# jinggqu/NextGen-UIA

Hardware: AMD Instinct MI355X
Metric: images/sec fwd+bwd BiomedCLIP+Mona bs=256 (higher is better)
Workload: dtype bf16

## Files before the change

### nextgen-uia_amd/csrc/gemm.hip

```cpp
#include "gemm_epilogue.h"

int uia_gemm_quad_launch(hipStream_t stream, const UiaGemmParams& p, bool specialise, int xflags);
int uia_gemm_quadv_launch(hipStream_t stream, const UiaGemmParams& p, bool specialise, int xflags, int depth);

namespace {

template <typename T, int BM, int BN, int WAVES_M, int WAVES_N>
__global__ __launch_bounds__(64 * WAVES_M * WAVES_N) void gemm_tn_kernel(const UiaGemmParams p) {
    extern __shared__ __attribute__((aligned(16))) char smem[];
    constexpr int NW = WAVES_M * WAVES_N;
    constexpr int WTM = BM / WAVES_M, WTN = BN / WAVES_N;
    constexpr int MT = WTM / 16, NT = WTN / 16;
    constexpr int A_BYTES = BM * 128, W_BYTES = BN * 128, BUF_BYTES = A_BYTES + W_BYTES;
    constexpr int A_PER_WAVE = (BM / 8) / NW, W_PER_WAVE = (BN / 8) / NW;
    static_assert((BM / 8) % NW == 0 && (BN / 8) % NW == 0, "staging must divide over the waves");
    static_assert(WTM % 16 == 0 && WTN % 16 == 0 && (NT % 2) == 0, "wave tile shape");
    constexpr int ESZ = (int)sizeof(T);

    const int tid = threadIdx.x, lane = tid & 63;
    const int wave = __builtin_amdgcn_readfirstlane(tid >> 6);
    const int wm = wave / WAVES_N, wn = wave % WAVES_N;

    const int tiles_n = (p.N + BN - 1) / BN;
    const int nwg = gridDim.x;
    int bid = blockIdx.x;
    {
// ... 1201 lines not shown
                  "uia_gemm: outT_kb_rows needs outT, at least M rows, N*sizeof(T) a multiple of 64 and no row remapping");
    UIA_CHECK_ARG(!p.resid_ln_stats || p.resid_ln_dim >= 0, "uia_gemm: resid_ln_dim=%d", p.resid_ln_dim);
    UIA_CHECK_ARG(!p.rowsum_out || ((uintptr_t)p.rowsum_out % 16 == 0 && p.out_group == 0), "uia_gemm: rowsum_out must be 16-byte aligned and takes no row remapping");
    UIA_CHECK_ARG(!(p.resid_ln_stats && p.resid_ln_dim > 0) || (uintptr_t)p.resid_ln_stats % 16 == 0, "uia_gemm: row sums behind resid_ln_stats must be 16-byte aligned");
    UIA_CHECK_ARG(!p.ln_flag || (uintptr_t)p.ln_flag % 4 == 0, "uia_gemm: ln_flag must be a 4-byte aligned device word");
    UIA_CHECK_ARG(p.drop_where >= 0 && p.drop_where <= 2, "uia_gemm: drop_where=%d (0 none, 1 A operand, 2 accumulator)", p.drop_where);
    UIA_CHECK_ARG(p.drop_where == 0 || (p.drop_p >= 0.f && p.drop_p < 1.f), "uia_gemm: drop_p=%f outside [0, 1)", (double)p.drop_p);
    UIA_CHECK_ARG(p.drop_where != 1 || (dtype == UIA_BF16 && (size_t)p.M * (size_t)p.K / 8 <= 0xFFFFFFFFull && (uintptr_t)p.a_drop_out % 16 == 0 && !p.a_kb_rows),
                  "uia_gemm: dropout on the A operand needs bf16, row-major A, M*K <= 2^35 and a 16-byte aligned a_drop_out");
    UIA_CHECK_ARG(p.drop_where != 2 || (size_t)p.M * (size_t)p.N / 8 <= 0xFFFFFFFFull, "uia_gemm: dropout on the accumulator needs M*N <= 2^35");
    UIA_CHECK_ARG(p.drop_where == 1 || !p.a_drop_out, "uia_gemm: a_drop_out without drop_where = 1");
    UIA_CHECK_ARG(p.K2 >= 0 && (p.K2 == 0 || (dtype == UIA_BF16 && p.A2 && p.K2 % 32 == 0 && p.K2 < p.K && p.lda2 >= p.K2 && (p.lda2 * 2) % 16 == 0 && (uintptr_t)p.A2 % 16 == 0 &&
                                             p.a2_group_cols >= 0 && p.a2_group_cols % 256 == 0 && !p.a_kb_rows && p.lda >= p.K - p.K2)),
                  "uia_gemm: the K extension needs bf16, a row-major A of K - K2 columns, a 16-byte aligned row-major A2 with K2 (a multiple of 32, < K) columns and "
                  "column groups that are multiples of 256; got K=%d K2=%d lda2=%lld group=%d", p.K, p.K2, (long long)p.lda2, p.a2_group_cols);
    UIA_CHECK_ARG(!p.lnfold_sums || (p.lnfold_colsum && p.lnfold_dim > 0 && p.alpha == 1.0f && (uintptr_t)p.lnfold_sums % 16 == 0 && (uintptr_t)p.lnfold_colsum % 16 == 0),
                  "uia_gemm: lnfold_sums needs lnfold_colsum (16-byte aligned), lnfold_dim > 0 and alpha == 1");
    UIA_CHECK_ARG(!p.outT || p.outT_kb_rows || p.ldo >= p.N, "uia_gemm: ldo=%lld < N=%d", (long long)p.ldo, p.N);
    UIA_CHECK_ARG(!p.out32 || p.ldo32 >= p.N, "uia_gemm: ldo32=%lld < N=%d", (long long)p.ldo32, p.N);
    UIA_CHECK_ARG(!p.aux_out || p.ldaux_out >= p.N, "uia_gemm: ldaux_out=%lld < N=%d", (long long)p.ldaux_out, p.N);
    UIA_CHECK_ARG(!p.aux_in || p.ldaux_in >= p.N, "uia_gemm: ldaux_in=%lld < N=%d", (long long)p.ldaux_in, p.N);
    UIA_CHECK_ARG(!p.resid || p.ldr >= p.N, "uia_gemm: ldr=%lld < N=%d", (long long)p.ldr, p.N);
    UIA_CHECK_ARG(!p.residT || p.residT_kb_rows || p.ldrT >= p.N, "uia_gemm: ldrT=%lld < N=%d", (long long)p.ldrT, p.N);
    if (dtype == UIA_BF16) return launch_typed<bf16_t>(stream, p, cfg);
    return launch_typed<float>(stream, p, cfg);
}
```

### nextgen-uia_amd/uia_hip/functional.py

```python
import math
import os
import weakref

import time

import torch

from . import handoff, ops
from ._lib import UiaError
from .handoff import (ClsGrad, Resid3, _g3_partner_feeds, cls_grad_of, fwd3_of, grad3_decode, grad3_of, grad_resid3_enabled, hook_free, linear_chain,
                      publish_cls_grad, publish_fwd3, publish_grad3, publish_rows, publish_t_copy, set_cls_grad, set_grad_resid3, t_copy_of, take_rows, zero_sums,
                      cls_only, set_cls_forward, take_cls_forward)
from .handoff import clear as clear_t_copies

_STATE = {"dtype": torch.bfloat16, "seed": 0x5EED, "calls": 0, "fwd_resid3": os.environ.get("UIA_FWD_RESID3", "1") != "0"}


def set_compute_dtype(dt):
    assert dt in (torch.bfloat16, torch.float32)
    _STATE["dtype"] = dt


def compute_dtype():
    return _STATE["dtype"]
# ... 300 lines not shown
WEIGHTS = WeightCache()


def _empty(shape, dt, like):
    return torch.empty(shape, device=like.device, dtype=dt)


def _act(M, K, dt, like, n_consumer):
    if ops.kb_ok(M, n_consumer, K, dt):
        return ops.kb_empty(M, K, dt, like.device)
    return torch.empty((M, K), device=like.device, dtype=dt)


def _attn_act(M, K, dt, like, n_consumer):
    return _act(M, K, dt, like, n_consumer) if dt == torch.bfloat16 else torch.empty((M, K), device=like.device, dtype=dt)


def _as_act(buf, M, K, dt, n_consumer):
    if ops.kb_ok(M, n_consumer, K, dt):
        return buf if ops.is_kb(buf) else ops.KBlocked.over(buf.view(M, K))
    return buf.as_rows() if ops.is_kb(buf) else buf


def _rows_tile_cfg(m_dense, w, like, dt, **facts):
    if dt != torch.float32 or not like.is_cuda:
        return 0
    N, K = (w.row if isinstance(w, ops.PackedW) else w).shape
    plan = ops.plan_gemm(m_dense, N, K, 4, ops.num_cus(like.device.index), 0, packed=isinstance(w, ops.PackedW), **facts)
    return next(L.base for L in plan if L.lo == 0)


MONA_PARAM_ORDER = ("gamma", "gammax", "project1.weight", "project1.bias", "project2.weight", "project2.bias", "norm.weight", "norm.bias",
                    "adapter_conv.conv1.weight", "adapter_conv.conv1.bias", "adapter_conv.conv2.weight", "adapter_conv.conv2.bias",
                    "adapter_conv.conv3.weight", "adapter_conv.conv3.bias", "adapter_conv.projector.weight", "adapter_conv.projector.bias",
                    "adapter_conv.freq_filter", "adapter_conv.noise_estimator.1.weight", "adapter_conv.noise_estimator.1.bias",
                    "adapter_conv.noise_estimator.3.weight", "adapter_conv.noise_estimator.3.bias")
_SPATIAL_MAP = {"adapter_conv.conv1.weight": "conv1_w", "adapter_conv.conv1.bias": "conv1_b", "adapter_conv.conv2.weight": "conv2_w",
                "adapter_conv.conv2.bias": "conv2_b", "adapter_conv.conv3.weight": "conv3_w", "adapter_conv.conv3.bias": "conv3_b",
                "adapter_conv.projector.weight": "proj_w", "adapter_conv.projector.bias": "proj_b", "adapter_conv.freq_filter": "freq",
                "adapter_conv.noise_estimator.1.weight": "ne1_w", "adapter_conv.noise_estimator.1.bias": "ne1_b",
                "adapter_conv.noise_estimator.3.weight": "ne3_w", "adapter_conv.noise_estimator.3.bias": "ne3_b"}


class MonaFn(torch.autograd.Function):

    @staticmethod
    def forward(ctx, x, variant, hw, p_drop, keep_mask, names, direct, *params):
        P = dict(zip(names, params))
        B, N, D = x.shape
# ... 8 lines not shown
        sp = {_SPATIAL_MAP[k]: v.detach().contiguous() for k, v in P.items() if k in _SPATIAL_MAP}
        seed = _next_seed() if (p_drop > 0 and keep_mask is None) else 0
        fold = not rows and ln_fold_enabled(dt, M)
        if not rows and ops.mona_fused_ok(dt, D, h, w, bott):
            train = any(ctx.needs_input_grad)
            u = _empty((M, D), dt, x) if train else None
            t = _empty((M, bott), dt, x) if train else None
            d = _empty((M, bott), dt, x) if train else None
            w1, w2 = WEIGHTS.get(P["project1.weight"], dt), WEIGHTS.get(P["project2.weight"], dt)
            y = torch.empty_like(x)
            y_t, sums = (_act(M, D, dt, x, 3 * D), zero_sums(M, x.device)) if fold else (None, None)
            ops.mona_fused_fwd(variant, B, h, w, x, P["norm.weight"], P["norm.bias"], P["gamma"], P["gammax"], w1.row, P["project1.bias"], w2.row,
                               P["project2.bias"], sp, y, y_t=y_t, rowsum=sums, u_out=u, t_out=t, d_out=d, p_drop=p_drop, seed=seed, keep_mask=keep_mask)
            if fold:
                publish_rows(y, y_t, sums)
        else:
            u = _empty((M, D), dt, x)
            w1 = WEIGHTS.get(P["project1.weight"], dt)
            t = _empty((M, bott), dt, x)
            if ops.MONA_PRE_FWD_T and x.is_cuda and dt == torch.bfloat16 and D == 768 and bott == 64:
                ops.mona_pre_fwd(x, P["norm.weight"], P["norm.bias"], P["gamma"], P["gammax"], u, proj1=(w1.row if isinstance(w1, ops.PackedW) else w1, P["project1.bias"], t))
            else:
                ops.mona_pre_fwd(x, P["norm.weight"], P["norm.bias"], P["gamma"], P["gammax"], u)
                ops.gemm(u, w1, bias=P["project1.bias"], out_t=t, tile_cfg=_rows_tile_cfg(B * ntok, w1, x, dt, out_t=True) if rows else 0)
            d = _empty((M, bott), dt, x)
            if rows:
                ops.mona_cls_fwd(B, ntok, t, d, p_drop=p_drop, seed=seed, keep_mask=keep_mask)
            else:
                ops.mona_spatial_fwd(variant, B, h, w, t, sp, d, p_drop=p_drop, seed=seed, keep_mask=keep_mask)
            w2 = WEIGHTS.get(P["project2.weight"], dt)
            y = torch.empty_like(x)
            y_t, sums = (_act(M, D, dt, x, 3 * D), zero_sums(M, x.device)) if fold else (None, None)
            three = fold and dt == torch.bfloat16 and _STATE.get("fwd_resid3", True) and handoff.fwd3_consumer_ahead() and M > 2048 and x.is_cuda
            y_lo = torch.empty(M, D, device=x.device, dtype=torch.int8) if three else None
            ops.gemm(d, w2, bias=P["project2.bias"], resid=x.view(M, D), out32=None if three else y.view(M, D), out_t=y_t, out_lo=y_lo, rowsum=sums,
                     tile_cfg=_rows_tile_cfg(B * ntok, w2, x, dt, out32=True, resid=True) if rows else 0)
            if three:
                y = publish_fwd3(x.shape, x.device, y_t, y_lo, sums)
            elif fold:
                publish_rows(y, y_t, sums)
        if u is not None:
            ctx.save_for_backward(x, u, t, d, keep_mask if keep_mask is not None else x.new_empty(0), *params)
        ctx.meta = (variant, hw, p_drop, seed, names, keep_mask is not None)
        ctx.direct_params = tuple(params) if direct else None
        ctx.g3_out = dt == torch.bfloat16 and _g3_partner_feeds(x)
        front = handoff.partner_node(x)
        ctx.cls_ok = not rows and u is not None and type(front).__name__ == "VitBlockFnBackward" and handoff.takes_cls_grad(x)
        ctx.rows_ntok = ntok if rows else 0
        return y

    @staticmethod
    def backward_cls(ctx, cg):
        ntok = getattr(ctx, "rows_ntok", 0)
        variant, hw, p_drop, seed, names, has_mask = ctx.meta
        x, u, t, d, keep_mask, *params = ctx.saved_tensors
        keep_mask = keep_mask if has_mask else None
        P = dict(zip(names, params))
        B, N, D = x.shape
        dt, bott = u.dtype, t.shape[1]
        dy = cg.rows32
        dy_t = dy if dt == torch.float32 else (cg.rows_t if cg.rows_t is not None else t_copy_of(dy, dt))
        direct = ctx.direct_params is not None and all(_is_flat_grad(p) for p in ctx.direct_params)
        G = ({k: p.grad for k, p in zip(names, ctx.direct_params)} if direct
             else {k: torch.zeros_like(v, dtype=torch.float32) for k, v in P.items()})
        cls_rows = lambda a: a.view(B, N * a.shape[1])[:, :a.shape[1]]
        side = _wgrad_side_stream(x.device) if _STATE.get("wgrad_side_stream", False) else None
        w2t = WEIGHTS.get(P["project2.weight"], dt, transpose=True)
        dd = _empty((B, bott), dt, x)
        _wgrad_beside(side, lambda: ops.gemm(dy_t, w2t, out_t=dd), dy_t, cls_rows(d), G["project2.weight"], G["project2.bias"])
        dtt = _empty((B, bott), dt, x)
        ops.mona_cls_bwd(B, ntok or N, dd, t, dtt, p_drop=p_drop, seed=seed, keep_mask=keep_mask, t_rows=bool(ntok))
        w1t = WEIGHTS.get(P["project1.weight"], dt, transpose=True)
        fuse_du = x.is_cuda and ops.mona_pre_bwd_du_ok(B, D, bott, dt)
        du = None if fuse_du else _empty((B, D), dt, x)
        _wgrad_beside(side, None if fuse_du else (lambda: ops.gemm(dtt, w1t, out_t=du)), dtt, cls_rows(u), G["project1.weight"], G["project1.bias"])
        need_dx = ctx.needs_input_grad[0]
        x_cls = x.view(B, D) if ntok else ops.copy_rows(x.view(B * N, D), N, _empty((B, D), torch.float32, x))
        dx = _empty((B, D), torch.float32, x) if need_dx else None
        dx_t = _empty((B, D), dt, x) if (need_dx and dt != torch.float32) else None
        w1t_rows = (dtt, w1t.row if isinstance(w1t, ops.PackedW) else w1t) if fuse_du else None
        ops.mona_pre_bwd(du, x_cls, dy if need_dx else None, P["norm.weight"], P["norm.bias"], P["gamma"], P["gammax"], dx, dx_t,
                         G["gamma"], G["gammax"], G["norm.weight"], G["norm.bias"], dt_w1t=w1t_rows)
        if need_dx and ntok:
            dx = dx.view(B, 1, D)
            publish_t_copy(dx, dx_t.view(B, 1, D) if dx_t is not None else None)
        elif need_dx:
            dx = publish_cls_grad(x.shape, x.device, dx, dx_t) if ctx.cls_ok else ClsGrad(dx, dx_t, N).decode()
        grads = tuple(None if direct else (G[k] if ctx.needs_input_grad[7 + i] else None) for i, k in enumerate(names))
        return (dx, None, None, None, None, None, None) + grads

    @staticmethod
    def backward(ctx, dy):
        if getattr(ctx, "rows_ntok", 0):
            dy = dy.contiguous()
            B, _, D = dy.shape
            dt = ctx.saved_tensors[1].dtype
            return MonaFn.backward_cls(ctx, ClsGrad(dy.view(B, D), t_copy_of(dy, dt).view(B, D) if dt != torch.float32 else None, ctx.rows_ntok))
        cg = cls_grad_of(dy)
# ... 186 lines not shown
            saved, ctx.layout = handoff.save_layout(x3.resid3 if x3 is not None else x, qkv, a, lse, Resid3(h1, lo1) if r3 else x1, pre)
            ctx.save_for_backward(*saved)
            ctx.xshape = (B, N, D)
            ctx.spec = spec
            ctx.g3_out = dt == torch.bfloat16 and _g3_partner_feeds(x)
            ctx.cls_ok = spec.mask is None and N <= ATTN_SINGLE_PASS_MAX and D == 64 * spec.heads and not r3 and handoff.cls_grad_enabled()
        return x2

    @staticmethod
    def _forward_cls(ctx, x, x3, qkv, spec, shape, dt, train):
        B, N, D = shape
        like = qkv
        a = _empty((B, D), dt, like)
        lse = torch.empty(B, spec.heads, device=like.device, dtype=torch.float32) if train else None
        ops.attn_fwd_cls(qkv[:, :D], qkv[:, D:2 * D], qkv[:, 2 * D:], a, B, spec.heads, N, lse=lse)
        x_cls = torch.empty(B, D, device=like.device, dtype=torch.float32)
        if x3 is not None:
            ops.rows3_to_f32(x3.hi, x3.lo, N, x_cls)
        else:
            ops.copy_rows(x.view(B * N, D), N, x_cls)
        x1 = torch.empty(B, D, device=like.device, dtype=torch.float32)
        M = B * N
        wp = WEIGHTS.get(spec.proj[0], dt)
        ops.gemm(a, wp, bias=spec.proj[1], resid=x_cls, out32=x1, tile_cfg=_rows_tile_cfg(M, wp, like, dt, out32=True, resid=True))
        h2 = _empty((B, D), dt, like)
        ops.layernorm_fwd(x1, spec.ln2[0], spec.ln2[1], spec.eps, y_t=h2)
        F = spec.fc1[0].shape[0]
        f = _empty((B, F), dt, like)
        pre = _empty((B, F), dt, like) if train else None
        w1, w2 = WEIGHTS.get(spec.fc1[0], dt), WEIGHTS.get(spec.fc2[0], dt)
        ops.gemm(h2, w1, bias=spec.fc1[1], act=spec.act, aux_out=pre, out_t=f, tile_cfg=_rows_tile_cfg(M, w1, like, dt, act=True, aux_out=train, out_t=True))
        x2 = torch.empty(B, 1, D, device=like.device, dtype=torch.float32)
        ops.gemm(f, w2, bias=spec.fc2[1], resid=x1, out32=x2.view(B, D), tile_cfg=_rows_tile_cfg(M, w2, like, dt, out32=True, resid=True))
        if train:
            saved, ctx.layout = handoff.save_layout(x3.resid3 if x3 is not None else x, qkv, a, lse, x1, pre)
            ctx.save_for_backward(*saved)
            ctx.xshape = (B, N, D)
            ctx.spec = spec
            ctx.g3_out = dt == torch.bfloat16 and _g3_partner_feeds(x)
            ctx.cls_ok = False
            ctx.cls_fwd = True
        handoff.cls_rows_out(True)
        return x2

    @staticmethod
    def backward_cls(ctx, cg):
        compact = getattr(ctx, "cls_fwd", False)
        xin, qkv, a, lse, x1, pre = handoff.restore_layout(ctx.saved_tensors, ctx.layout)
        x3_in = isinstance(xin, Resid3)
        x = xin.lo if x3_in else xin
        spec = ctx.spec
        B, N, D = ctx.xshape
        M, dt = B * N, qkv.dtype
        F = pre.shape[1]
        dy = cg.rows32
        dy_t = dy if dt == torch.float32 else (cg.rows_t if cg.rows_t is not None else t_copy_of(dy, dt))
        pre_cls = pre if compact else ops.copy_rows(pre, N, _empty((B, F), dt, x))
        dpre = _empty((B, F), dt, x)
        ops.gemm(dy_t, WEIGHTS.get(spec.fc2[0], dt, transpose=True), dact=spec.act, aux_in=pre_cls, out_t=dpre)
        dh = _empty((B, D), dt, x)
        ops.gemm(dpre, WEIGHTS.get(spec.fc1[0], dt, transpose=True), out_t=dh)
        x1_cls = x1 if compact else ops.copy_rows(x1, N, _empty((B, D), torch.float32, x))
        dx1 = _empty((B, D), torch.float32, x)
        dx1_t = _empty((B, D), dt, x) if dt != torch.float32 else dx1
        ops.layernorm_bwd(dh, x1_cls, spec.ln2[0], spec.eps, dres=dy, dx32=dx1, dx_t=dx1_t if dt != torch.float32 else None)
        da = dh
        ops.gemm(dx1_t, WEIGHTS.get(spec.proj[0], dt, transpose=True), out_t=da)
        dqkv = _attn_act(M, 3 * D, dt, x, D)
        if ops.is_kb(dqkv):
            ops.attn_bwd_cls(qkv[:, :D], qkv[:, D:2 * D], qkv[:, 2 * D:], a, da, lse, dqkv, None, None, B, spec.heads, N, rows=compact)
        else:
            ops.attn_bwd_cls(qkv[:, :D], qkv[:, D:2 * D], qkv[:, 2 * D:], a, da, lse, dqkv[:, :D], dqkv[:, D:2 * D], dqkv[:, 2 * D:], B, spec.heads, N, rows=compact)
        dh1 = _empty((M, D), dt, x)
        ops.gemm(dqkv, WEIGHTS.get(spec.qkv[0], dt, transpose=True), out_t=dh1)
        xrows = xin if x3_in else x.view(M, D)
        if getattr(ctx, "g3_out", False):
            dx_t = _empty((M, D), dt, x)
            dlo = torch.empty(M, D, device=x.device, dtype=torch.int8)
            ops.layernorm_bwd_periodic(dh1, xrows, spec.ln1[0], spec.eps, dx1, N, dx_t=dx_t, dx_lo=dlo)
            return publish_grad3((B, N, D), x.device, dx_t, dlo), None
        dx = torch.empty(B, N, D, device=x.device, dtype=torch.float32)
        if dt == torch.float32:
            ops.layernorm_bwd_periodic(dh1, xrows, spec.ln1[0], spec.eps, dx1, N, dx32=dx.view(M, D))
            return dx, None
        dx_t = _empty((M, D), dt, x)
        ops.layernorm_bwd(dh1, xrows, spec.ln1[0], spec.eps, dres=ClsGrad(dx1, None, N).decode().view(M, D), dx32=dx.view(M, D), dx_t=dx_t)
        publish_t_copy(dx, dx_t)
        return dx, None

    @staticmethod
# ... 99 lines not shown
    rows = torch.empty(B, D, device=res.w.device, dtype=torch.float32)
    if res.lo is not None:
        ops.rows3_to_f32(res.hi, res.lo, L, rows)
    else:
        ops.copy_rows(res.raw.view(-1, D), L, rows)
        if res.stats is None:
            return rows
    ops.layernorm_fwd(rows, res.w, res.b, res.eps if res.eps is not None else eps, y32=rows)
    return rows


def post_ln_layer_cls_ok(x_t, heads, L, cu_seqlens=None):
    D = x_t.cols if ops.is_kb(x_t) else x_t.shape[1]
    return cu_seqlens is None and D == 64 * heads and 1 < L <= 288 and x_t.is_cuda and not (x_t.dtype != torch.float32 and _STATE.get("text_resid_t", False))


def _post_ln_layer_cls(res, qkv, L, B, heads, P, keylen, eps, D, dt):
    a = _empty((B, D), dt, qkv)
    ops.attn_fwd_cls(qkv[:, :D], qkv[:, D:2 * D], qkv[:, 2 * D:], a, B, heads, L, mask="keypad", keylen=keylen)
    r = _res_cls_rows(res, L, B, D, eps)
    s_a = torch.empty(B, D, device=qkv.device, dtype=torch.float32)
    M = B * L
    wo = WEIGHTS.get(P["attention.output.dense.weight"], dt)
    ops.gemm(a, wo, bias=P["attention.output.dense.bias"], resid=r, out32=s_a, tile_cfg=_rows_tile_cfg(M, wo, qkv, dt, out32=True, resid=True))
    h = _empty((B, D), dt, qkv)
    ops.layernorm_fwd(s_a, P["attention.output.LayerNorm.weight"], P["attention.output.LayerNorm.bias"], eps, y_t=h, y32=s_a)
    F = P["intermediate.dense.weight"].shape[0]
    f = _empty((B, F), dt, qkv)
    w1, w2 = WEIGHTS.get(P["intermediate.dense.weight"], dt), WEIGHTS.get(P["output.dense.weight"], dt)
    ops.gemm(h, w1, bias=P["intermediate.dense.bias"], act="gelu", out_t=f, tile_cfg=_rows_tile_cfg(M, w1, qkv, dt, act=True, out_t=True))
    ops.gemm(f, w2, bias=P["output.dense.bias"], resid=s_a, out32=r, tile_cfg=_rows_tile_cfg(M, w2, qkv, dt, out32=True, resid=True))
    ops.layernorm_fwd(r, P["output.LayerNorm.weight"], P["output.LayerNorm.bias"], eps, y_t=h, y32=r)
    return LnResidual(r, None, P["output.LayerNorm.weight"], P["output.LayerNorm.bias"]), h


def post_ln_layer(res, x_t, L, B, heads, P, keylen, eps=1e-12, cu_seqlens=None, fold_sums=None, fold_out=False, cls_only=False):
    kb_in = ops.is_kb(x_t)
    M, D = (x_t.rows, x_t.cols) if kb_in else x_t.shape
    dt = x_t.dtype
    t_resid = dt != torch.float32 and _STATE.get("text_resid_t", False)
    fold = fold_sums is not None and ln_fold_enabled(dt, M) and not t_resid
    qkv = _empty((M, 3 * D), dt, x_t)
    if res.dim is not None:
        wq, cq, bq = WEIGHTS.get_lnfold(P["_qkv_raw"][0], P["_qkv_raw"][1], res.w, res.b, dt)
        ops.gemm(x_t, wq, bias=bq, out_t=qkv, lnfold=(res.stats, cq, D, res.eps))
    else:
        ops.gemm(x_t, P["_qkv_w"](dt), bias=P["_qkv_b"], out_t=qkv)
    if cls_only:
        return _post_ln_layer_cls(res, qkv, L, B, heads, P, keylen, eps, D, dt)
    a = _attn_act(M, D, dt, x_t, D) if (D == 64 * heads and cu_seqlens is None) else _empty((M, D), dt, x_t)
    if cu_seqlens is not None:
        ops.attn_fwd(qkv[:, :D], qkv[:, D:2 * D], qkv[:, 2 * D:], a, B, heads, L, cu_seqlens=cu_seqlens)
    else:
        ops.attn_fwd(qkv[:, :D], qkv[:, D:2 * D], qkv[:, 2 * D:], a, B, heads, L, mask="keypad", keylen=keylen)
# ... 1217 lines not shown
```

### nextgen-uia_amd/uia_hip/ops.py

```python
import ctypes as C
from typing import NamedTuple

import torch

from . import _lib
from ._lib import AttnDesc, GemmDesc, LnLoraDesc, LoraRankDesc, MonaFusedDesc, MonaSpatialDesc, PackDesc, UiaError, WgradGroupDesc, check, lib

_ACT = {None: 0, "none": 0, "gelu": 1, "quick_gelu": 2, "relu": 3}

GEMM_PROFILE = None


EPI_BIAS, EPI_AUX_OUT, EPI_GELU, EPI_DGELU, EPI_RESID, EPI_RESIDT, EPI_OUT32, EPI_OUTT, EPI_RESID_LN, EPI_GENERIC = 1, 2, 4, 8, 16, 32, 64, 128, 256, -1
EPI_QUICK = 2048
EPI_ROWSUM, EPI_LNFOLD = 512, 1024
EPI_RESID_LO, EPI_OUT_LO = 4096, 8192
_SPECIALISED = {EPI_BIAS | EPI_RESID | EPI_OUT32, EPI_BIAS | EPI_RESIDT | EPI_OUT32, EPI_BIAS | EPI_RESID | EPI_RESID_LN | EPI_OUT32, EPI_OUTT, EPI_BIAS | EPI_OUTT, EPI_BIAS | EPI_GELU | EPI_OUTT, EPI_DGELU | EPI_OUTT,
                EPI_BIAS | EPI_GELU | EPI_AUX_OUT | EPI_OUTT,
                EPI_QUICK | EPI_BIAS | EPI_GELU | EPI_OUTT, EPI_QUICK | EPI_DGELU | EPI_OUTT, EPI_QUICK | EPI_BIAS | EPI_GELU | EPI_AUX_OUT | EPI_OUTT,
                EPI_BIAS | EPI_RESID | EPI_OUT32 | EPI_OUTT | EPI_ROWSUM, EPI_BIAS | EPI_RESID | EPI_RESID_LN | EPI_OUT32 | EPI_OUTT | EPI_ROWSUM,
                EPI_BIAS | EPI_OUTT | EPI_LNFOLD, EPI_BIAS | EPI_GELU | EPI_OUTT | EPI_LNFOLD, EPI_BIAS | EPI_GELU | EPI_AUX_OUT | EPI_OUTT | EPI_LNFOLD,
                EPI_QUICK | EPI_BIAS | EPI_GELU | EPI_OUTT | EPI_LNFOLD, EPI_QUICK | EPI_BIAS | EPI_GELU | EPI_AUX_OUT | EPI_OUTT | EPI_LNFOLD,
                EPI_BIAS | EPI_RESID_LO | EPI_RESID_LN | EPI_OUTT | EPI_OUT_LO | EPI_ROWSUM,
                EPI_BIAS | EPI_RESID | EPI_OUTT | EPI_OUT_LO | EPI_ROWSUM, EPI_BIAS | EPI_RESID_LO | EPI_OUT32,
# ... 65 lines not shown
    dev = torch.cuda.current_device() if device is None else device
    if dev not in _NCU:
        _NCU[dev] = torch.cuda.get_device_properties(dev).multi_processor_count
    return _NCU[dev]


def big_tile_cfg(N, K, esz):
    if QUAD and esz == 2:
        return 25
    if QUADV and esz == 2:
        return QUADV if QUADV in (27, 29) else 27
    return 24 if (RING5 and esz == 2 and (K * esz >= 2048 or N >= 2304)) else 8


def tail_k_slices(rows, N, K, esz, ncu):
    tiles = -(-rows // 128) * -(-N // 256)
    kb = K * esz
    if not TAIL_SPLIT_K or esz != 2 or kb < 4096 or 4 * tiles > ncu:
        return 0
    s = min(ncu // tiles, kb // 1024, 16)
    return s if s >= 2 else 0


def splitk_workspace(floats, device):
    key = (device.index if device.index is not None else torch.cuda.current_device(), torch.cuda.current_stream(device).cuda_stream)
    t = _SPLITK_WS.get(key)
    if t is None or t.numel() < floats:
        t = _SPLITK_WS[key] = torch.zeros(max(floats, 1 << 20), device=device, dtype=torch.float32)
    return t


class _TailFork:

    def __init__(self, device):
        self.cur = torch.cuda.current_stream(device)
        key = (device.index if device.index is not None else torch.cuda.current_device(), self.cur.cuda_stream)
        e = _TAIL_SIDE.get(key)
        if e is None:
            e = _TAIL_SIDE[key] = (torch.cuda.Stream(device=device), torch.cuda.Event(), torch.cuda.Event())
        self.side, self.ev_in, self.ev_out = e
        self.ctx = None

    def __enter__(self):
        self.ev_in.record(self.cur)
        self.side.wait_event(self.ev_in)
        self.ctx = torch.cuda.stream(self.side)
        self.ctx.__enter__()
        return self

    def __exit__(self, *exc):
        self.ev_out.record(self.side)
        self.ctx.__exit__(*exc)
# ... 270 lines not shown


_F32, _FT = (torch.float32,), (torch.bfloat16, torch.float32)


def _rowmajor(t, name):
    if t.dim() != 2 or t.stride(1) != 1:
        raise UiaError(f"{name} must be a 2-D row-major tensor (got shape {tuple(t.shape)}, stride {t.stride()})")
    return t.stride(0)


class Launch(NamedTuple):
    lo: int
    hi: int
    tile_cfg: int
    base: int
    w_kblocked: bool
    side: bool
    scratch: int


def plan_gemm(M, N, K, esz, ncu, tile_cfg=0, *, whole=False, ext=False, packed=False, on_device=True, out_group=0, resid_mod=0, drop=None, alpha=1.0,
              a_kb=False, out_t_kb=False, act=False, aux_out=False, out_t=False, out32=False, resid=False, resid_t=False, rowsum=False, ln=False):
    auto = 0 if (ext or tile_cfg & 255) else auto_tile_cfg(M, N, K, esz)

    def launch(lo, hi, word, side=False, scratch=0):
        base = word & 255
        if ext:
            if not base:
                base = 8 if hi - lo > 2048 else 13
                word |= base
        elif not base:
            base = auto
            if (base == 14 and esz == 2 and K == 64 and N % 64 == 0 and N * 144 <= 160 * 1024 and not (a_kb or out_t_kb or act or aux_out or rowsum or ln)
                    and out_group == 0 and resid_mod == 0 and drop in (None, "acc")
                    and ((out_t and not out32 and not resid and (resid_t or drop is not None)) or (out32 and not out_t and not resid_t and (resid or drop is not None)))):
                base = 23
            elif base == 8:
                base = big_tile_cfg(N, K, esz)
                word |= base
        if PERSIST_STORE_ONLY and base == 8 and not (resid or resid_t or out32 or rowsum) and out_group == 0 and alpha == 1.0 and K * esz >= 1024:
            base, word = 12, (word & ~255) | 12
        if TILE_GROUP and N in TILE_GROUP and (word >> 8) == 0 and base in RING_CFGS:
            word |= int(TILE_GROUP[N]) << 8
        return Launch(lo, hi, word, base, bool(ext or (packed and KBLOCK_W and base in RING_CFGS and on_device)), side, scratch)

# ... 124 lines not shown
            d.a_drop_out = _p(xo)
    packed = w if isinstance(w, PackedW) else None
    if ext is not None:
        d.lda, d.ldw, d.M, d.K, d.N = _rowmajor(a, "a"), ext.K, a.shape[0], ext.K, ext.N
        d.A = _p(a)
    else:
        wrow = packed.row if packed is not None else w
        d.ldw = _rowmajor(wrow, "w")
        if is_kb(a):
            d.M, d.K, d.a_kb_rows = _kb_dims(a, "gemm a")
            d.lda = d.K
        else:
            d.lda = _rowmajor(a, "a")
            d.M, d.K = a.shape[0], a.shape[1]
        if a.dtype != wrow.dtype or d.K != wrow.shape[1]:
            raise UiaError(f"gemm operand mismatch: a {(d.M, d.K)} {a.dtype}, w {tuple(wrow.shape)} {wrow.dtype}")
        d.A = _p(a.t if is_kb(a) else a)
        d.N = wrow.shape[0]
    esz = a.element_size()
    if launch is None:
        launch = plan_gemm(d.M, d.N, d.K, esz, 0, tile_cfg, whole=True,
                           **_plan_facts(a, w, act, dact, aux_out, out_group, resid_mod, drop, alpha, out_t, out32, resid, resid_t, rowsum, lnfold, resid_ln))[0]
    tile_cfg, base_cfg = launch.tile_cfg, launch.base
    d.W, d.w_kblocked = (_p(ext.kb if ext is not None else packed.kblocked()), 1) if launch.w_kblocked else (_p(wrow), 0)
    d.alpha = alpha
    d.act, d.dact = _ACT[act], _ACT[dact]
    if bias is not None:
        assert bias.dtype == torch.float32 and bias.numel() == d.N
        d.bias = _p(bias)
    for name, t, want in (("aux_in", aux_in, a.dtype), ("aux_out", aux_out, a.dtype), ("resid_t", resid_t, a.dtype),
                          ("resid", resid, torch.float32), ("out32", out32, torch.float32)):
        if t is not None and t.dtype != want:
            raise UiaError(f"gemm {name} must be {want}, got {t.dtype}")
    for name, t in (("aux_in", aux_in), ("aux_out", aux_out), ("resid_t", resid_t), ("out32", out32)):
        if t is not None and (t.dim() != 2 or t.shape[1] < d.N or (t.shape[0] < d.M and out_group == 0)):
            raise UiaError(f"gemm {name} is {tuple(t.shape)}: too small for the [{d.M}, {d.N}] result")
    if resid is not None and resid_mod == 0 and out_group == 0 and (resid.dim() != 2 or resid.shape[1] < d.N or resid.shape[0] < d.M):
        raise UiaError(f"gemm resid is {tuple(resid.shape)}: too small for the [{d.M}, {d.N}] result")
    if aux_in is not None:
        d.aux_in, d.ldaux_in = _p(aux_in), _rowmajor(aux_in, "aux_in")
    if aux_out is not None:
        d.aux_out, d.ldaux_out = _p(aux_out), _rowmajor(aux_out, "aux_out")
    if resid is not None:
        d.resid, d.ldr = _p(resid), _rowmajor(resid, "resid")
    d.resid_mod, d.resid_row_off, d.out_group = resid_mod, resid_row_off, out_group
    if resid_ln is not None:
# ... 1447 lines not shown
```

Measured before the change: 6762.

## Add split-K small-M rows GEMM kernel for CLS-only bf16 GEMMs

```diff
diff --git a/nextgen-uia_amd/csrc/gemm.hip b/nextgen-uia_amd/csrc/gemm.hip
--- a/nextgen-uia_amd/csrc/gemm.hip
+++ b/nextgen-uia_amd/csrc/gemm.hip
@@ -2,6 +2,7 @@
 
 int uia_gemm_quad_launch(hipStream_t stream, const UiaGemmParams& p, bool specialise, int xflags);
 int uia_gemm_quadv_launch(hipStream_t stream, const UiaGemmParams& p, bool specialise, int xflags, int depth);
+int uia_gemm_rows_launch(hipStream_t stream, int dtype, const UiaGemmParams& p, int slices_req);
 
 namespace {
 
@@ -1249,6 +1250,7 @@
     UIA_CHECK_ARG(!p.aux_in || p.ldaux_in >= p.N, "uia_gemm: ldaux_in=%lld < N=%d", (long long)p.ldaux_in, p.N);
     UIA_CHECK_ARG(!p.resid || p.ldr >= p.N, "uia_gemm: ldr=%lld < N=%d", (long long)p.ldr, p.N);
     UIA_CHECK_ARG(!p.residT || p.residT_kb_rows || p.ldrT >= p.N, "uia_gemm: ldrT=%lld < N=%d", (long long)p.ldrT, p.N);
+    if ((cfg & 255) == 30) return uia_gemm_rows_launch(stream, dtype, p, (cfg >> 16) & 63);
     if (dtype == UIA_BF16) return launch_typed<bf16_t>(stream, p, cfg);
     return launch_typed<float>(stream, p, cfg);
 }
diff --git a/nextgen-uia_amd/csrc/gemm_rows.hip b/nextgen-uia_amd/csrc/gemm_rows.hip
--- /dev/null
+++ b/nextgen-uia_amd/csrc/gemm_rows.hip
@@ -0,0 +1,241 @@
+#include "gemm_epilogue.h"
+
+namespace {
+
+constexpr int ROWS_TICKET_WORDS = 1024;
+constexpr int ROWS_MAX_SLICES = 32;
+
+int rows_auto_slices(int rows, int blocks, int N, int K, int ncu) {
+    const int strips = (N / 64) * blocks, ksteps = K / 64;
+    const int step_ns = 27 * (rows + 64) / 32, slab_ns = rows * 256 / 100;
+    int best = 1, best_cost = ksteps * step_ns;
+    for (int s = 2; s <= ksteps && s <= ROWS_MAX_SLICES && s * strips <= (ncu > strips ? ncu : strips); ++s) {
+        const int per = (ksteps + s - 1) / s;
+        if ((ksteps + per - 1) / per != s) continue;
+        const int cost = per * step_ns + 1700 + slab_ns * 6 / 10 + s * slab_ns;
+        if (cost < best_cost) { best = s; best_cost = cost; }
+    }
+    return best;
+}
+
+template <int GPT>
+__device__ __forceinline__ void wait_all_but(int steps) {
+    switch (steps) {
+        case 0: asm volatile("s_waitcnt vmcnt(0)" ::: "memory"); break;
+        case 1: asm volatile("s_waitcnt vmcnt(%0)" ::"n"(GPT) : "memory"); break;
+        case 2: asm volatile("s_waitcnt vmcnt(%0)" ::"n"(2 * GPT) : "memory"); break;
+        case 3: asm volatile("s_waitcnt vmcnt(%0)" ::"n"(3 * GPT) : "memory"); break;
+        case 4: asm volatile("s_waitcnt vmcnt(%0)" ::"n"(4 * GPT) : "memory"); break;
+        case 5: asm volatile("s_waitcnt vmcnt(%0)" ::"n"(5 * GPT) : "memory"); break;
+        default: asm volatile("s_waitcnt vmcnt(%0)" ::"n"(6 * GPT) : "memory"); break;
+    }
+}
+
+template <int MT>
+__global__ __launch_bounds__(256) void gemm_rows_kernel(const UiaGemmParams p, const int slices, const int per_slice) {
+    extern __shared__ __attribute__((aligned(16))) char smem[];
+    using T = bf16_t;
+    constexpr int NW = 4, BM = 64 * MT, BN = 64, WTM = 16 * MT, NT = 4;
+    constexpr int NBUF = MT == 1 ? 8 : 6;
+    constexpr int A_BYTES = BM * 128, W_BYTES = BN * 128, BUF_BYTES = A_BYTES + W_BYTES;
+    constexpr int A_PER_WAVE = (BM / 8) / NW, W_PER_WAVE = (BN / 8) / NW, GPT = A_PER_WAVE + W_PER_WAVE;
+    static_assert(NBUF - 2 <= 6 && (NBUF - 2) * GPT < 64, "the counted waits");
+
+    const int tid = threadIdx.x, lane = tid & 63;
+    const int wave = __builtin_amdgcn_readfirstlane(tid >> 6);
+
+    int bid = blockIdx.x;
+    {
+        const int nwg = gridDim.x, xcd = bid & 7, q = nwg >> 3, r = nwg & 7;
+        bid = (xcd < r ? xcd * (q + 1) : r * (q + 1) + (xcd - r) * q) + (bid >> 3);
+    }
+    const int tile = bid / slices, slice = bid - tile * slices;
+    const int blocks = (p.M + BM - 1) / BM;
+    const int strip = tile / blocks, m0 = (tile - strip * blocks) * BM;
+    const int n0 = strip * BN;
+    const int ksteps = p.K / 64;
+    const int k0 = slice * per_slice;
+    const int nk = (k0 + per_slice <= ksteps ? per_slice : ksteps - k0);
+
+    const char* srcA[A_PER_WAVE];
+    const char* srcW[W_PER_WAVE];
+#pragma unroll
+    for (int i = 0; i < A_PER_WAVE; ++i) {
+        const int r = 8 * (wave + NW * i) + (lane >> 3);
+        const int c = (lane & 7) ^ ((r >> 1) & 7);
+        const int gm = m0 + r < p.M ? m0 + r : p.M - 1;
+        srcA[i] = (const char*)p.A + ((size_t)gm * (size_t)p.lda + (size_t)k0 * 64) * 2 + c * 16;
+    }
+#pragma unroll
+    for (int i = 0; i < W_PER_WAVE; ++i) {
+        const int r = 8 * (wave + NW * i) + (lane >> 3);
+        const int x = ((r / (4 * NT)) << 1) | ((r & 3) >> 1);
+        const int c = (lane & 7) ^ x;
+        srcW[i] = (const char*)p.W + ((size_t)(n0 + r) * (size_t)p.ldw + (size_t)k0 * 64) * 2 + c * 16;
+    }
+
+    const int li = lane & 15, g = lane >> 4;
+    const int offA0 = (wave * WTM + li) * 128 + ((g ^ (li >> 1)) << 4);
+    const int xw = ((li >> 2) << 1) | ((li & 3) >> 1);
+    const int offW0 = A_BYTES + ((li >> 2) * (4 * NT) + (li & 3)) * 128 + ((g ^ xw) << 4);
+
+    f32x4 acc[MT][NT];
+#pragma unroll
+    for (int i = 0; i < MT; ++i)
+#pragma unroll
+        for (int j = 0; j < NT; ++j) acc[i][j] = f32x4{0.f, 0.f, 0.f, 0.f};
+
+    auto stage = [&](int s, int buf) {
+        char* base = smem + buf * BUF_BYTES;
+        const size_t koff = (size_t)s * 128;
+#pragma unroll
+        for (int i = 0; i < A_PER_WAVE; ++i) glds16_asm(srcA[i] + koff, base + (wave + NW * i) * 1024);
+#pragma unroll
+        for (int i = 0; i < W_PER_WAVE; ++i) glds16_asm(srcW[i] + koff, base + A_BYTES + (wave + NW * i) * 1024);
+    };
+
+    for (int s = 0; s < NBUF - 1 && s < nk; ++s) stage(s, s);
+    int cur = 0;
+    for (int s = 0; s < nk; ++s) {
+        const int behind = nk - 1 - s;
+        wait_all_but<GPT>(behind < NBUF - 2 ? behind : NBUF - 2);
+        __syncthreads();
+        if (s + NBUF - 1 < nk) stage(s + NBUF - 1, cur == 0 ? NBUF - 1 : cur - 1);
+        const char* buf = smem + cur * BUF_BYTES;
+#pragma unroll
+        for (int kk = 0; kk < 2; ++kk) {
+            uint4 af[MT], wf[NT];
+#pragma unroll
+            for (int j = 0; j < NT; ++j) wf[j] = *(const uint4*)(buf + ((offW0 + j * 4 * 128) ^ (kk << 6)));
+#pragma unroll
+            for (int i = 0; i < MT; ++i) af[i] = *(const uint4*)(buf + ((offA0 + i * 16 * 128) ^ (kk << 6)));
+#pragma unroll
+            for (int i = 0; i < MT; ++i)
+#pragma unroll
+                for (int j = 0; j < NT; ++j) acc[i][j] = MfmaTile<T>::mma(wf[j], af[i], acc[i][j]);
+        }
+        cur = cur == NBUF - 1 ? 0 : cur + 1;
+    }
+
+    if (slices > 1) {
+        unsigned* tickets = (unsigned*)p.splitk_ws;
+        float* slabs = p.splitk_ws + ROWS_TICKET_WORDS;
+        const size_t slab_floats = (size_t)BM * BN;
+        const size_t strip_base = (size_t)tile * slices * slab_floats;
+        {
+            float* mine = slabs + strip_base + (size_t)slice * slab_floats + tid * 4;
+#pragma unroll
+            for (int i = 0; i < MT; ++i) {
+                if (m0 + wave * WTM + 16 * i < p.M) {
+#pragma unroll
+                    for (int j = 0; j < NT; ++j) *(f32x4*)(mine + (i * NT + j) * 1024) = acc[i][j];
+                }
+            }
+        }
+        asm volatile("s_waitcnt vmcnt(0)" ::: "memory");
+        __syncthreads();
+        int* last_flag = (int*)smem;
+        if (tid == 0) {
+            __builtin_amdgcn_fence(__ATOMIC_RELEASE, "agent");
+            asm volatile("s_waitcnt vmcnt(0)" ::: "memory");
+            const unsigned t = __hip_atomic_fetch_add(tickets + tile, 1u, __ATOMIC_RELAXED, __HIP_MEMORY_SCOPE_AGENT);
+            const int last = t == (unsigned)(slices - 1);
+            if (last) {
+                __builtin_amdgcn_fence(__ATOMIC_ACQUIRE, "agent");
+                asm volatile("s_waitcnt vmcnt(0)" ::: "memory");
+                __hip_atomic_store(tickets + tile, 0u, __ATOMIC_RELAXED, __HIP_MEMORY_SCOPE_AGENT);
+            }
+            *last_flag = last;
+        }
+        __syncthreads();
+        if (!*last_flag) return;
+        const float* all = slabs + strip_base + tid * 4;
+#pragma unroll
+        for (int i = 0; i < MT; ++i)
+#pragma unroll
+            for (int j = 0; j < NT; ++j) acc[i][j] = f32x4{0.f, 0.f, 0.f, 0.f};
+#pragma unroll 2
+        for (int s = 0; s < slices; ++s) {
+            const float* sl = all + (size_t)s * slab_floats;
+#pragma unroll
+            for (int i = 0; i < MT; ++i) {
+                if (m0 + wave * WTM + 16 * i < p.M) {
+#pragma unroll
+                    for (int j = 0; j < NT; ++j) acc[i][j] += *(const f32x4*)(sl + (i * NT + j) * 1024);
+                }
+            }
+        }
+    }
+
+    T* outT = (T*)p.outT;
+    const T* aux_in = (const T*)p.aux_in;
+    T* aux_out = (T*)p.aux_out;
+#pragma unroll
+    for (int i = 0; i < MT; ++i) {
+        const size_t m = (size_t)(m0 + wave * WTM + 16 * i + li);
+        if (m >= (size_t)p.M) continue;
+#pragma unroll
+        for (int jj = 0; jj < NT; jj += 2) {
+            const int n = n0 + g * 16 + 4 * jj;
+            float v[8];
+#pragma unroll
+            for (int e = 0; e < 4; ++e) { v[e] = acc[i][jj][e]; v[4 + e] = acc[i][jj + 1][e]; }
+            if (p.bias) {
+                float b[8];
+                load8(p.bias + n, b);
+#pragma unroll
+                for (int e = 0; e < 8; ++e) v[e] += b[e];
+            }
+            if (aux_out) store8(aux_out + m * p.ldaux_out + n, v);
+            if (p.act) apply_act8<true>(v, p.act);
+            if (p.dact) {
+                float a[8];
+                load8(aux_in + m * p.ldaux_in + n, a);
+                apply_dact8<true>(v, a, p.dact);
+            }
+            if (p.resid) {
+                float r[8];
+                load8(p.resid + m * p.ldr + n, r);
+#pragma unroll
+                for (int e = 0; e < 8; ++e) v[e] += r[e];
+            }
+            if (p.out32) store8(p.out32 + m * p.ldo32 + n, v);
+            if (outT) store8(outT + m * p.ldo + n, v);
+        }
+    }
+}
+
+template <int MT>
+int launch_rows(hipStream_t stream, const UiaGemmParams& p, int slices, int per_slice) {
+    constexpr int LDS = (MT == 1 ? 8 : 6) * (64 * MT + 64) * 128;
+    auto kern = gemm_rows_kernel<MT>;
+    static UiaDevOnce attr_once;
+    UIA_ENSURE_LDS_ATTR(attr_once, kern, LDS);
+    hipLaunchKernelGGL(kern, dim3((p.N / 64) * ((p.M + 64 * MT - 1) / (64 * MT)) * slices), dim3(256), LDS, stream, p, slices, per_slice);
+    UIA_CHECK_LAUNCH();
+    return 0;
+}
+
+}
+
+int uia_gemm_rows_launch(hipStream_t stream, int dtype, const UiaGemmParams& p, int slices_req) {
+    UIA_CHECK_ARG(dtype == UIA_BF16, "uia_gemm: tile cfg 30 (small-M rows kernel) is bf16 only");
+    UIA_CHECK_ARG(p.M >= 1 && p.M <= 256, "uia_gemm: tile cfg 30 takes 1 <= M <= 256, got M=%d", p.M);
+    UIA_CHECK_ARG(p.N % 64 == 0 && p.K % 64 == 0, "uia_gemm: tile cfg 30 needs N and K to be multiples of 64, got N=%d K=%d", p.N, p.K);
+    UIA_CHECK_ARG(p.N / 64 <= ROWS_TICKET_WORDS / 2, "uia_gemm: tile cfg 30 takes N <= %d", 32 * ROWS_TICKET_WORDS);
+    UIA_CHECK_ARG(!p.a_kb_rows && !p.outT_kb_rows && !p.w_kblocked, "uia_gemm: tile cfg 30 takes row-major operands and outputs (no K-blocked A, W or outT)");
+    UIA_CHECK_ARG(p.alpha == 1.0f && p.resid_mod == 0 && p.out_group == 0 && !p.residT && !p.resid_ln_stats && !p.rowsum_out && !p.lnfold_sums &&
+                      p.drop_where == 0 && p.K2 == 0 && !p.A2 && !p.resid_lo8 && !p.out_lo8,
+                  "uia_gemm: tile cfg 30 runs bias, act + aux_out, dact + aux_in, fp32 resid, out32 and outT only (no alpha, row remapping, residT, LayerNorm fold, "
+                  "row sums, dropout, K extension or three-byte tensors)");
+    const int rows = p.M <= 64 ? 64 : 128, blocks = (p.M + rows - 1) / rows, ksteps = p.K / 64;
+    int slices = slices_req > 0 ? slices_req : rows_auto_slices(rows, blocks, p.N, p.K, uia_num_cus());
+    UIA_CHECK_ARG(slices <= ROWS_MAX_SLICES, "uia_gemm: tile cfg 30 takes at most %d K slices, got %d", ROWS_MAX_SLICES, slices);
+    if (slices > ksteps) slices = ksteps;
+    const int per_slice = (ksteps + slices - 1) / slices;
+    slices = (ksteps + per_slice - 1) / per_slice;
+    UIA_CHECK_ARG(slices == 1 || (p.splitk_ws && (uintptr_t)p.splitk_ws % 16 == 0),
+                  "uia_gemm: tile cfg 30 with %d K slices needs a 16-byte aligned splitk_ws (%d ticket words, zero, + slices x N x %d floats)", slices, ROWS_TICKET_WORDS,
+                  rows * blocks);
+    return rows == 64 ? launch_rows<1>(stream, p, slices, per_slice) : launch_rows<2>(stream, p, slices, per_slice);
+}
diff --git a/nextgen-uia_amd/uia_hip/functional.py b/nextgen-uia_amd/uia_hip/functional.py
--- a/nextgen-uia_amd/uia_hip/functional.py
+++ b/nextgen-uia_amd/uia_hip/functional.py
@@ -346,9 +346,16 @@
     return buf.as_rows() if ops.is_kb(buf) else buf
 
 
-def _rows_tile_cfg(m_dense, w, like, dt, **facts):
+def _rows_gemm_cfg(rows, w, like, dt):
+    if dt != torch.bfloat16 or not like.is_cuda:
+        return 0
+    N, K = (w.row if isinstance(w, ops.PackedW) else w).shape
+    return ops.ROWS_CFG if ops.rows_gemm_ok(rows, N, K, 2) else 0
+
+
+def _rows_tile_cfg(m_dense, w, like, dt, rows=0, **facts):
     if dt != torch.float32 or not like.is_cuda:
-        return 0
+        return _rows_gemm_cfg(rows, w, like, dt) if rows else 0
     N, K = (w.row if isinstance(w, ops.PackedW) else w).shape
     plan = ops.plan_gemm(m_dense, N, K, 4, ops.num_cus(like.device.index), 0, packed=isinstance(w, ops.PackedW), **facts)
     return next(L.base for L in plan if L.lo == 0)
@@ -403,7 +410,7 @@
                 ops.mona_pre_fwd(x, P["norm.weight"], P["norm.bias"], P["gamma"], P["gammax"], u, proj1=(w1.row if isinstance(w1, ops.PackedW) else w1, P["project1.bias"], t))
             else:
                 ops.mona_pre_fwd(x, P["norm.weight"], P["norm.bias"], P["gamma"], P["gammax"], u)
-                ops.gemm(u, w1, bias=P["project1.bias"], out_t=t, tile_cfg=_rows_tile_cfg(B * ntok, w1, x, dt, out_t=True) if rows else 0)
+                ops.gemm(u, w1, bias=P["project1.bias"], out_t=t, tile_cfg=_rows_tile_cfg(B * ntok, w1, x, dt, rows=B, out_t=True) if rows else 0)
             d = _empty((M, bott), dt, x)
             if rows:
                 ops.mona_cls_fwd(B, ntok, t, d, p_drop=p_drop, seed=seed, keep_mask=keep_mask)
@@ -415,7 +422,7 @@
             three = fold and dt == torch.bfloat16 and _STATE.get("fwd_resid3", True) and handoff.fwd3_consumer_ahead() and M > 2048 and x.is_cuda
             y_lo = torch.empty(M, D, device=x.device, dtype=torch.int8) if three else None
             ops.gemm(d, w2, bias=P["project2.bias"], resid=x.view(M, D), out32=None if three else y.view(M, D), out_t=y_t, out_lo=y_lo, rowsum=sums,
-                     tile_cfg=_rows_tile_cfg(B * ntok, w2, x, dt, out32=True, resid=True) if rows else 0)
+                     tile_cfg=_rows_tile_cfg(B * ntok, w2, x, dt, rows=B, out32=True, resid=True) if rows else 0)
             if three:
                 y = publish_fwd3(x.shape, x.device, y_t, y_lo, sums)
             elif fold:
@@ -448,13 +455,13 @@
         side = _wgrad_side_stream(x.device) if _STATE.get("wgrad_side_stream", False) else None
         w2t = WEIGHTS.get(P["project2.weight"], dt, transpose=True)
         dd = _empty((B, bott), dt, x)
-        _wgrad_beside(side, lambda: ops.gemm(dy_t, w2t, out_t=dd), dy_t, cls_rows(d), G["project2.weight"], G["project2.bias"])
+        _wgrad_beside(side, lambda: ops.gemm(dy_t, w2t, out_t=dd, tile_cfg=_rows_gemm_cfg(B, w2t, x, dt)), dy_t, cls_rows(d), G["project2.weight"], G["project2.bias"])
         dtt = _empty((B, bott), dt, x)
         ops.mona_cls_bwd(B, ntok or N, dd, t, dtt, p_drop=p_drop, seed=seed, keep_mask=keep_mask, t_rows=bool(ntok))
         w1t = WEIGHTS.get(P["project1.weight"], dt, transpose=True)
         fuse_du = x.is_cuda and ops.mona_pre_bwd_du_ok(B, D, bott, dt)
         du = None if fuse_du else _empty((B, D), dt, x)
-        _wgrad_beside(side, None if fuse_du else (lambda: ops.gemm(dtt, w1t, out_t=du)), dtt, cls_rows(u), G["project1.weight"], G["project1.bias"])
+        _wgrad_beside(side, None if fuse_du else (lambda: ops.gemm(dtt, w1t, out_t=du, tile_cfg=_rows_gemm_cfg(B, w1t, x, dt))), dtt, cls_rows(u), G["project1.weight"], G["project1.bias"])
         need_dx = ctx.needs_input_grad[0]
         x_cls = x.view(B, D) if ntok else ops.copy_rows(x.view(B * N, D), N, _empty((B, D), torch.float32, x))
         dx = _empty((B, D), torch.float32, x) if need_dx else None
@@ -687,16 +694,16 @@
         x1 = torch.empty(B, D, device=like.device, dtype=torch.float32)
         M = B * N
         wp = WEIGHTS.get(spec.proj[0], dt)
-        ops.gemm(a, wp, bias=spec.proj[1], resid=x_cls, out32=x1, tile_cfg=_rows_tile_cfg(M, wp, like, dt, out32=True, resid=True))
+        ops.gemm(a, wp, bias=spec.proj[1], resid=x_cls, out32=x1, tile_cfg=_rows_tile_cfg(M, wp, like, dt, rows=B, out32=True, resid=True))
         h2 = _empty((B, D), dt, like)
         ops.layernorm_fwd(x1, spec.ln2[0], spec.ln2[1], spec.eps, y_t=h2)
         F = spec.fc1[0].shape[0]
         f = _empty((B, F), dt, like)
         pre = _empty((B, F), dt, like) if train else None
         w1, w2 = WEIGHTS.get(spec.fc1[0], dt), WEIGHTS.get(spec.fc2[0], dt)
-        ops.gemm(h2, w1, bias=spec.fc1[1], act=spec.act, aux_out=pre, out_t=f, tile_cfg=_rows_tile_cfg(M, w1, like, dt, act=True, aux_out=train, out_t=True))
+        ops.gemm(h2, w1, bias=spec.fc1[1], act=spec.act, aux_out=pre, out_t=f, tile_cfg=_rows_tile_cfg(M, w1, like, dt, rows=B, act=True, aux_out=train, out_t=True))
         x2 = torch.empty(B, 1, D, device=like.device, dtype=torch.float32)
-        ops.gemm(f, w2, bias=spec.fc2[1], resid=x1, out32=x2.view(B, D), tile_cfg=_rows_tile_cfg(M, w2, like, dt, out32=True, resid=True))
+        ops.gemm(f, w2, bias=spec.fc2[1], resid=x1, out32=x2.view(B, D), tile_cfg=_rows_tile_cfg(M, w2, like, dt, rows=B, out32=True, resid=True))
         if train:
             saved, ctx.layout = handoff.save_layout(x3.resid3 if x3 is not None else x, qkv, a, lse, x1, pre)
             ctx.save_for_backward(*saved)
@@ -722,15 +729,17 @@
         dy_t = dy if dt == torch.float32 else (cg.rows_t if cg.rows_t is not None else t_copy_of(dy, dt))
         pre_cls = pre if compact else ops.copy_rows(pre, N, _empty((B, F), dt, x))
         dpre = _empty((B, F), dt, x)
-        ops.gemm(dy_t, WEIGHTS.get(spec.fc2[0], dt, transpose=True), dact=spec.act, aux_in=pre_cls, out_t=dpre)
+        w2t, w1t = WEIGHTS.get(spec.fc2[0], dt, transpose=True), WEIGHTS.get(spec.fc1[0], dt, transpose=True)
+        ops.gemm(dy_t, w2t, dact=spec.act, aux_in=pre_cls, out_t=dpre, tile_cfg=_rows_gemm_cfg(B, w2t, x, dt))
         dh = _empty((B, D), dt, x)
-        ops.gemm(dpre, WEIGHTS.get(spec.fc1[0], dt, transpose=True), out_t=dh)
+        ops.gemm(dpre, w1t, out_t=dh, tile_cfg=_rows_gemm_cfg(B, w1t, x, dt))
         x1_cls = x1 if compact else ops.copy_rows(x1, N, _empty((B, D), torch.float32, x))
         dx1 = _empty((B, D), torch.float32, x)
         dx1_t = _empty((B, D), dt, x) if dt != torch.float32 else dx1
         ops.layernorm_bwd(dh, x1_cls, spec.ln2[0], spec.eps, dres=dy, dx32=dx1, dx_t=dx1_t if dt != torch.float32 else None)
         da = dh
-        ops.gemm(dx1_t, WEIGHTS.get(spec.proj[0], dt, transpose=True), out_t=da)
+        wpt = WEIGHTS.get(spec.proj[0], dt, transpose=True)
+        ops.gemm(dx1_t, wpt, out_t=da, tile_cfg=_rows_gemm_cfg(B, wpt, x, dt))
         dqkv = _attn_act(M, 3 * D, dt, x, D)
         if ops.is_kb(dqkv):
             ops.attn_bwd_cls(qkv[:, :D], qkv[:, D:2 * D], qkv[:, 2 * D:], a, da, lse, dqkv, None, None, B, spec.heads, N, rows=compact)
@@ -876,14 +885,14 @@
     s_a = torch.empty(B, D, device=qkv.device, dtype=torch.float32)
     M = B * L
     wo = WEIGHTS.get(P["attention.output.dense.weight"], dt)
-    ops.gemm(a, wo, bias=P["attention.output.dense.bias"], resid=r, out32=s_a, tile_cfg=_rows_tile_cfg(M, wo, qkv, dt, out32=True, resid=True))
+    ops.gemm(a, wo, bias=P["attention.output.dense.bias"], resid=r, out32=s_a, tile_cfg=_rows_tile_cfg(M, wo, qkv, dt, rows=B, out32=True, resid=True))
     h = _empty((B, D), dt, qkv)
     ops.layernorm_fwd(s_a, P["attention.output.LayerNorm.weight"], P["attention.output.LayerNorm.bias"], eps, y_t=h, y32=s_a)
     F = P["intermediate.dense.weight"].shape[0]
     f = _empty((B, F), dt, qkv)
     w1, w2 = WEIGHTS.get(P["intermediate.dense.weight"], dt), WEIGHTS.get(P["output.dense.weight"], dt)
-    ops.gemm(h, w1, bias=P["intermediate.dense.bias"], act="gelu", out_t=f, tile_cfg=_rows_tile_cfg(M, w1, qkv, dt, act=True, out_t=True))
-    ops.gemm(f, w2, bias=P["output.dense.bias"], resid=s_a, out32=r, tile_cfg=_rows_tile_cfg(M, w2, qkv, dt, out32=True, resid=True))
+    ops.gemm(h, w1, bias=P["intermediate.dense.bias"], act="gelu", out_t=f, tile_cfg=_rows_tile_cfg(M, w1, qkv, dt, rows=B, act=True, out_t=True))
+    ops.gemm(f, w2, bias=P["output.dense.bias"], resid=s_a, out32=r, tile_cfg=_rows_tile_cfg(M, w2, qkv, dt, rows=B, out32=True, resid=True))
     ops.layernorm_fwd(r, P["output.LayerNorm.weight"], P["output.LayerNorm.bias"], eps, y_t=h, y32=r)
     return LnResidual(r, None, P["output.LayerNorm.weight"], P["output.LayerNorm.bias"]), h
 
diff --git a/nextgen-uia_amd/uia_hip/ops.py b/nextgen-uia_amd/uia_hip/ops.py
--- a/nextgen-uia_amd/uia_hip/ops.py
+++ b/nextgen-uia_amd/uia_hip/ops.py
@@ -111,12 +111,50 @@
     return s if s >= 2 else 0
 
 
-def splitk_workspace(floats, device):
+def splitk_workspace(floats, device, rows=False):
     key = (device.index if device.index is not None else torch.cuda.current_device(), torch.cuda.current_stream(device).cuda_stream)
-    t = _SPLITK_WS.get(key)
+    pool = _ROWS_WS if rows else _SPLITK_WS
+    t = pool.get(key)
     if t is None or t.numel() < floats:
-        t = _SPLITK_WS[key] = torch.zeros(max(floats, 1 << 20), device=device, dtype=torch.float32)
+        t = pool[key] = torch.zeros(max(floats, 1 << 20), device=device, dtype=torch.float32)
     return t
+
+
+ROWS_CFG = 30
+ROWS_TICKET_WORDS = 1024
+ROWS_MAX_SLICES = 32
+_ROWS_WS = {}
+
+
+def rows_gemm_rows(M):
+    return 64 if M <= 64 else 128
+
+
+def rows_gemm_slices(M, N, K, ncu):
+    rows = rows_gemm_rows(M)
+    blocks = -(-M // rows)
+    strips, ksteps = N // 64 * blocks, K // 64
+    step_ns, slab_ns = 27 * (rows + 64) // 32, rows * 256 // 100
+    best, best_cost = 1, ksteps * step_ns
+    s = 2
+    while s <= ksteps and s <= ROWS_MAX_SLICES and s * strips <= max(ncu, strips):
+        per = -(-ksteps // s)
+        if -(-ksteps // per) == s:
+            cost = per * step_ns + 1700 + slab_ns * 6 // 10 + s * slab_ns
+            if cost < best_cost:
+                best, best_cost = s, cost
+        s += 1
+    return best
+
+
+def rows_gemm_fit(K, slices):
+    ksteps = K // 64
+    per = -(-ksteps // max(1, min(slices, ksteps, ROWS_MAX_SLICES)))
+    return -(-ksteps // per)
+
+
+def rows_gemm_ok(M, N, K, esz):
+    return esz == 2 and 1 <= M <= 256 and N % 64 == 0 and K % 64 == 0 and N // 64 <= ROWS_TICKET_WORDS // 2
 
 
 class _TailFork:
@@ -433,6 +471,9 @@
 
 def plan_gemm(M, N, K, esz, ncu, tile_cfg=0, *, whole=False, ext=False, packed=False, on_device=True, out_group=0, resid_mod=0, drop=None, alpha=1.0,
               a_kb=False, out_t_kb=False, act=False, aux_out=False, out_t=False, out32=False, resid=False, resid_t=False, rowsum=False, ln=False):
+    if tile_cfg & 255 == ROWS_CFG:
+        s = rows_gemm_fit(K, (tile_cfg >> 16) & 63 or rows_gemm_slices(M, N, K, ncu or 256))
+        return [Launch(0, M, ROWS_CFG | s << 16, ROWS_CFG, False, False, ROWS_TICKET_WORDS + s * N * -(-M // rows_gemm_rows(M)) * rows_gemm_rows(M) if s > 1 else 0)]
     auto = 0 if (ext or tile_cfg & 255) else auto_tile_cfg(M, N, K, esz)
 
     def launch(lo, hi, word, side=False, scratch=0):
@@ -603,6 +644,8 @@
         launch = plan_gemm(d.M, d.N, d.K, esz, 0, tile_cfg, whole=True,
                            **_plan_facts(a, w, act, dact, aux_out, out_group, resid_mod, drop, alpha, out_t, out32, resid, resid_t, rowsum, lnfold, resid_ln))[0]
     tile_cfg, base_cfg = launch.tile_cfg, launch.base
+    if base_cfg == ROWS_CFG and launch.scratch and splitk_ws is None:
+        d.splitk_ws = _p(splitk_workspace(launch.scratch, a.device, rows=True))
     d.W, d.w_kblocked = (_p(ext.kb if ext is not None else packed.kblocked()), 1) if launch.w_kblocked else (_p(wrow), 0)
     d.alpha = alpha
     d.act, d.dact = _ACT[act], _ACT[dact]
```

New measurement: 6761. Within noise of the previous version (-0.0%).
